# theophile-lt/gpt2-vision-language

Hardware: AMD Instinct MI355X
Metric: training tokens/sec/node, GPT-2-124M seq1024; caption-step images/sec (higher is better)
Workload: dtype bf16; 1 GPU; gpt2-124m-lm-pretrain; micro_batch=16, seq_len=1024, grad_accum=32, global_batch=512, model=gpt2-124m, parallelism=dp1

## Files before the change

gpt2-vision-language_amd/csrc/gemm_pp3.h:

```cpp
#pragma once
#include "common.h"
#include "capi_util.h"
#include "gemm_common.h"
#include "gemm_ring.h"
#include "../../include/gvl.h"

namespace {

using namespace gvl_ring;

template <int PER, int MAXN, int X>
GVL_DEV void wait_vm_steps_x(int n) {
  if (MAXN >= 4 && n >= 4) { asm volatile("s_waitcnt vmcnt(%0)" ::"n"(4 * PER + X) : "memory"); return; }
  if (MAXN >= 3 && n == 3) { asm volatile("s_waitcnt vmcnt(%0)" ::"n"(3 * PER + X) : "memory"); return; }
  if (MAXN >= 2 && n == 2) { asm volatile("s_waitcnt vmcnt(%0)" ::"n"(2 * PER + X) : "memory"); return; }
  if (MAXN >= 1 && n == 1) { asm volatile("s_waitcnt vmcnt(%0)" ::"n"(1 * PER + X) : "memory"); return; }
  asm volatile("s_waitcnt vmcnt(%0)" ::"n"(X) : "memory");
}

constexpr uint32_t CNT_OOB = 0x7FFFFFF0u;
constexpr int CNT_NT = 18;
template <int EPI>
struct CntEpi {
  using KD = EpiKind<EPI>;
  static constexpr bool ON = EPI != EPI_GEN && !KD::AUX && !KD::DROP;
};
template <int FM, int FN, int EPI>
constexpr int cnt_stores() {
  return FM * (FN / 2 + FN % 2) * (EpiKind<EPI>::ACT ? 2 : 1);
}
typedef uint32_t cnt_u32x2 __attribute__((ext_vector_type(2)));
GVL_DEV uint32_t cnt_off(bool ok, int64_t byte_off) {
  uint32_t o = ok ? (uint32_t)byte_off : CNT_OOB;
  asm volatile("" : "+v"(o));
  return o;
}
typedef uint32_t cnt_u32x4 __attribute__((ext_vector_type(4)));

template <int FN>
GVL_DEV void cnt_bias(uint32_t a, uint2 (&bv)[FN]);
template <>
GVL_DEV void cnt_bias<3>(uint32_t a, uint2 (&bv)[3]) {
  asm volatile("ds_read_b64 %0, %3\n\tds_read_b64 %1, %3 offset:32\n\tds_read_b64 %2, %3 offset:64\n\t"
               "s_waitcnt lgkmcnt(0)"
               : "=&v"(bv[0]), "=&v"(bv[1]), "=&v"(bv[2])
               : "v"(a));
}
template <>
GVL_DEV void cnt_bias<4>(uint32_t a, uint2 (&bv)[4]) {
  asm volatile("ds_read_b64 %0, %4\n\tds_read_b64 %1, %4 offset:32\n\tds_read_b64 %2, %4 offset:64\n\t"
               "ds_read_b64 %3, %4 offset:96\n\ts_waitcnt lgkmcnt(0)"
               : "=&v"(bv[0]), "=&v"(bv[1]), "=&v"(bv[2]), "=&v"(bv[3])
               : "v"(a));
}

template <int FM, int FN, int EPI, int AUX>
GVL_DEV void gemm_epilogue_cnt(const GemmP& p, const float4_t (&acc)[FM][FN], int64_t mw0,
                               int64_t nw0, int lane, float alpha, uint32_t bias_lds,
                               __amdgpu_buffer_rsrc_t rc, __amdgpu_buffer_rsrc_t rp) {
  using KD = EpiKind<EPI>;
  const int q = lane >> 4;
  uint2 bv[FN];
#pragma unroll
  for (int j = 0; j < FN; ++j) bv[j] = make_uint2(0, 0);
  if constexpr (KD::BIAS) cnt_bias<FN>(bias_lds + (uint32_t)(2 * (nw0 + 4 * q)), bv);
  const uint2 z = make_uint2(0, 0);
#pragma unroll
  for (int i = 0; i < FM; ++i) {
    const int64_t m = mw0 + i * 16 + (lane & 15);
    const bool mok = m < p.M;
#pragma unroll
    for (int j = 0; j + 1 < FN; j += 2) {
      const int64_t n0 = nw0 + j * 16 + 4 * q, n1 = n0 + 16;
      float v0[4], v1[4], h0[4] = {0.f, 0.f, 0.f, 0.f}, h1[4] = {0.f, 0.f, 0.f, 0.f};
      gemm_epi_vals_k<EPI>(p, acc[i][j], m, n0, alpha, 1.f, bv[j], z, v0, h0);
      gemm_epi_vals_k<EPI>(p, acc[i][j + 1], m, n1, alpha, 1.f, bv[j + 1], z, v1, h1);
      const auto sx = __builtin_amdgcn_permlane16_swap(pack2(v0[0], v0[1]), pack2(v1[0], v1[1]), false, false);
      const auto sy = __builtin_amdgcn_permlane16_swap(pack2(v0[2], v0[3]), pack2(v1[2], v1[3]), false, false);
      const int64_t n = nw0 + 16 * (j + (q & 1)) + 8 * (q >> 1);
      const bool ok = mok && n < p.N;
      __builtin_amdgcn_raw_buffer_store_b128(cnt_u32x4{sx[0], sy[0], sx[1], sy[1]}, rc,
                                             cnt_off(ok, (m * p.ldc + n) * 2), 0, AUX);
      if constexpr (KD::ACT) {
        const auto hx = __builtin_amdgcn_permlane16_swap(pack2(h0[0], h0[1]), pack2(h1[0], h1[1]), false, false);
        const auto hy = __builtin_amdgcn_permlane16_swap(pack2(h0[2], h0[3]), pack2(h1[2], h1[3]), false, false);
        __builtin_amdgcn_raw_buffer_store_b128(cnt_u32x4{hx[0], hy[0], hx[1], hy[1]}, rp,
                                               cnt_off(ok, (m * p.ldp + n) * 2), 0, AUX);
      }
    }
    if constexpr (FN % 2 == 1) {
      constexpr int j = FN - 1;
      const int64_t n0 = nw0 + j * 16 + 4 * q;
      float v0[4], h0[4] = {0.f, 0.f, 0.f, 0.f};
      gemm_epi_vals_k<EPI>(p, acc[i][j], m, n0, alpha, 1.f, bv[j], z, v0, h0);
      const bool ok = mok && n0 < p.N;
      __builtin_amdgcn_raw_buffer_store_b64(cnt_u32x2{pack2(v0[0], v0[1]), pack2(v0[2], v0[3])}, rc,
                                            cnt_off(ok, (m * p.ldc + n0) * 2), 0, AUX);
      if constexpr (KD::ACT)
        __builtin_amdgcn_raw_buffer_store_b64(cnt_u32x2{pack2(h0[0], h0[1]), pack2(h0[2], h0[3])}, rp,
                                              cnt_off(ok, (m * p.ldp + n0) * 2), 0, AUX);
    }
  }
}

template <int BN, bool BMN>
struct SlabB {
  using type = Step<256, BMN, 8>;
};
template <bool BMN>
struct SlabB<192, BMN> {
  using type = Step192<BMN>;
};

template <int NS, bool AMN, bool BMN, int EPI, int BN = 256, int BM = 256>
__global__ __launch_bounds__(512, 1) void gemm_pp3_kernel(GemmP p) {
  constexpr int NW = 8, FM = BM / 32, FN = BN / 64;
  static_assert(NS >= 3 && NS <= 6, "ring geometry");
  static_assert(BN == 256 || BN == 192, "tile width");
  static_assert(BM == 256 || BM == 128, "tile height");
  using SA = Step<BM, AMN, NW>;
  using SB = typename SlabB<BN, BMN>::type;
  constexpr int SLOT = SA::BYTES + SB::BYTES;
  constexpr int IPW0 = SA::PER + SB::PER;
  constexpr int IPW1 = SA::PER + (BN == 256 ? SB::PER : 1);
  extern __shared__ __attribute__((aligned(16))) char smem[];
  const int tid = threadIdx.x, lane = tid & 63;
  const int wave = __builtin_amdgcn_readfirstlane(tid >> 6);
  const int g = wave >> 2, wc = wave & 3;

  const int per_batch = p.tiles_m * p.tiles_n * p.splits;
  const int total = per_batch * p.batch;
  const int G = gridDim.x, b = blockIdx.x;
  const int ntl = (total - b + G - 1) / G;
  const int nks = (int)(p.kper / KS);
  const int nsteps = ntl * nks;
  auto tile_coords = [&](int t, int64_t& m0, int64_t& n0, int64_t& k0, int& split, int& bi) {
    const int vid = b + t * G;
    const int q8 = total >> 3, r8 = total & 7, xcd = vid & 7;
    int work = (xcd < r8 ? xcd * (q8 + 1) : r8 * (q8 + 1) + (xcd - r8) * q8) + (vid >> 3);
    bi = work / per_batch;
    work -= bi * per_batch;
    int tm, tn;
    gemm_tile_of(work, p.splits, p.tiles_m, p.tiles_n, p.group, split, tm, tn);
    m0 = (int64_t)tm * BM;
    n0 = (int64_t)tn * BN;
    k0 = (int64_t)split * p.kper;
  };

  const int64_t a_rows = AMN ? p.K : p.M, b_rows = BMN ? p.K : p.N;
  __amdgpu_buffer_rsrc_t ra = uniform_rsrc(p.A, a_rows * p.lda * 2);
  __amdgpu_buffer_rsrc_t rb = uniform_rsrc(p.B, b_rows * p.ldb * 2);
  const int sa_step = SA::step_bytes(p.lda), sb_step = SB::step_bytes(p.ldb);
  int is_t = 0, is_k = 0;
  int offa[SA::PER], offb[SB::PER];
  {
    int64_t m0, n0, k0;
    int sp, bi;
    tile_coords(0, m0, n0, k0, sp, bi);
    if (p.batch > 1) {
      ra = uniform_rsrc(p.Ab[bi], a_rows * p.lda * 2);
      rb = uniform_rsrc(p.Bb[bi], b_rows * p.ldb * 2);
    }
    SA::base_offsets(p.lda, m0, k0, wave, lane, offa);
    SB::base_offsets(p.ldb, n0, k0, wave, lane, offb);
  }

#define GVL_PP3_ISSUE(gstep)                                                        \
  do {                                                                              \
    if ((gstep) < nsteps) {                                                         \
      char* slot_ = smem + ((gstep) % NS) * SLOT;                                   \
      SA::issue_at(ra, offa, is_k * sa_step, slot_, wave);                          \
      SB::issue_at(rb, offb, is_k * sb_step, slot_ + SA::BYTES, wave);              \
      if (++is_k == nks) {                                                          \
        is_k = 0;                                                                   \
        if (++is_t < ntl) {                                                         \
          int64_t m0_, n0_, k0_;                                                    \
          int sp_, bi_;                                                             \
          tile_coords(is_t, m0_, n0_, k0_, sp_, bi_);                               \
          if (p.batch > 1) {                                                        \
            ra = uniform_rsrc(p.Ab[bi_], a_rows * p.lda * 2);                       \
            rb = uniform_rsrc(p.Bb[bi_], b_rows * p.ldb * 2);                       \
          }                                                                         \
          SA::base_offsets(p.lda, m0_, k0_, wave, lane, offa);                      \
          SB::base_offsets(p.ldb, n0_, k0_, wave, lane, offb);                      \
        }                                                                           \
      }                                                                             \
    }                                                                               \
  } while (0)

  float4_t acc[FM][FN];
#pragma unroll
  for (int i = 0; i < FM; ++i)
#pragma unroll
    for (int j = 0; j < FN; ++j) acc[i][j] = float4_t{0.f, 0.f, 0.f, 0.f};

  const int arow = g * (BM / 2), bcol = wc * (BN / 4);
  constexpr bool DB = EPI == EPI_RES && AMN && BMN;
  constexpr int FPW = FM / 4 > 0 ? FM / 4 : 1;
  float4_t bacc[DB ? FPW : 1];
#pragma unroll
  for (int k = 0; k < (DB ? FPW : 1); ++k) bacc[k] = float4_t{0.f, 0.f, 0.f, 0.f};
  short8_t ones;
#pragma unroll
  for (int k = 0; k < 8; ++k) ones[k] = (short)0x3F80;
  bool do_db = false;
  constexpr bool CNT = CntEpi<EPI>::ON;
  constexpr int CNT_S = cnt_stores<FM, FN, EPI>();
  static_assert(!CNT || (NS - 2) * (IPW0 > IPW1 ? IPW0 : IPW1) + CNT_S <= 63, "vmcnt range");
  const bool cnt_on = CNT && p.cnt;
  const uint32_t bias_lds = (uint32_t)(NS * SLOT);
  const __amdgpu_buffer_rsrc_t rc_cnt = uniform_rsrc(p.C, CNT ? p.M * p.ldc * 2 : 0);
  const __amdgpu_buffer_rsrc_t rp_cnt =
      uniform_rsrc(EpiKind<EPI>::ACT ? p.pre_out : p.C, CNT && EpiKind<EPI>::ACT ? p.M * p.ldp * 2 : 0);
  if constexpr (CNT && EpiKind<EPI>::BIAS) {
    if (cnt_on)
      for (int n = tid * 8; n < p.N; n += 512 * 8)
        *reinterpret_cast<uint4*>(smem + NS * SLOT + 2 * n) = *reinterpret_cast<const uint4*>(p.bias + n);
  }
  int cnt_w = 0;
  float alpha = p.alpha;
  if (p.alpha_ptr) alpha *= *p.alpha_ptr;
#pragma unroll
  for (int i = 0; i < NS - 1; ++i) GVL_PP3_ISSUE(i);
  {
    const int r = nsteps - 1, n = r < 0 ? 0 : (r < NS - 2 ? r : NS - 2);
    if (g == 0) wait_vm_steps<IPW0, NS - 2>(n);
    else wait_vm_steps<IPW1, NS - 2>(n);
  }
  barrier_lds();
  if (g == 1) __builtin_amdgcn_s_barrier();

  int cu_t = 0, cu_k = 0;
  int64_t cu_m0, cu_n0, cu_k0;
  int cu_sp, cu_bi;
  tile_coords(0, cu_m0, cu_n0, cu_k0, cu_sp, cu_bi);
  EpiPre<FM, FN, EPI> pre;
  if (!cnt_on) pre.load_bias(p, cu_n0 + bcol, lane);
  if constexpr (DB) do_db = p.batch > 1 && p.splits == 1 && cu_n0 == 0 && p.Db[cu_bi] != nullptr;
#define GVL_PP3_EPILOGUE()                                                                   \
  do {                                                                                       \
    bool epi_ = true;                                                                        \
    if (p.splits == 2 && p.tickets != nullptr) {     \
         \
      const int tile_ = (cu_bi * p.tiles_m + (int)(cu_m0 / BM)) * p.tiles_n + (int)(cu_n0 / BN); \
      const int64_t pofs_ = (int64_t)cu_bi * 2 * p.M * p.N;                                  \
      const __amdgpu_buffer_rsrc_t rw = uniform_rsrc(p.ws + pofs_, p.ws_bytes - pofs_ * 4);   \
      epi_ = gemm_splitk_arrive<FM, FN>(p, acc, cu_sp, tile_, wave, cu_m0 + arow,            \
                                        cu_n0 + bcol, lane, rw);                             \
      if (epi_) gemm_splitk_gather<FM, FN>(p, acc, cu_sp, cu_m0 + arow, cu_n0 + bcol, lane, rw); \
    } else if (p.splits > 1) {                                                               \
      gemm_store_partial<FM, FN>(p, acc, cu_sp, cu_m0 + arow, cu_n0 + bcol, lane);           \
      epi_ = false;                                                                          \
    }                                                                                        \
    if (epi_) {                                                                              \
      void* c_ = p.batch > 1 ? p.Cb[cu_bi] : p.C;                                           \
      if (CNT && cnt_on) {                                                                   \
        if (p.st_nt)                                                                         \
          gemm_epilogue_cnt<FM, FN, EPI, CNT_NT>(p, acc, cu_m0 + arow, cu_n0 + bcol, lane, alpha, \
                                                 bias_lds, rc_cnt, rp_cnt);                  \
        else                                                                                 \
          gemm_epilogue_cnt<FM, FN, EPI, 0>(p, acc, cu_m0 + arow, cu_n0 + bcol, lane, alpha,  \
                                            bias_lds, rc_cnt, rp_cnt);                       \
        cnt_w = NS - 2;                                                                      \
      } else {                                                                               \
        gemm_epilogue16<FM, FN, EPI>(p, acc, cu_m0 + arow, cu_n0 + bcol, lane, alpha, pre, c_, \
                                     p.batch > 1 ? static_cast<const bf16_t*>(c_) : p.residual); \
      }                                                                                      \
    }                                                                                        \
    if constexpr (DB) {                                                                      \
      if (do_db && (lane >> 4) == 0) {                                                       \
        bf16_t* db_ = static_cast<bf16_t*>(p.Db[cu_bi]);                                     \
        _Pragma("unroll") for (int k = 0; k < FPW; ++k) {                                    \
          const int64_t m_ = cu_m0 + arow + 16 * (wc * FPW + k) + lane;                      \
          if (m_ < p.M) db_[m_] = f2bf(bf2f(db_[m_]) + bacc[k][0] * alpha);                  \
        }                                                                                    \
      }                                                                                      \
      _Pragma("unroll") for (int k = 0; k < FPW; ++k) bacc[k] = float4_t{0.f, 0.f, 0.f, 0.f}; \
    }                                                                                        \
  } while (0)

  short8_t af[FM], bf[FN];
  for (int c = 0; c < nsteps; ++c) {
    if (cu_k == 0 && c > 0) {
      GVL_PP3_EPILOGUE();
#pragma unroll
      for (int i = 0; i < FM; ++i)
#pragma unroll
        for (int j = 0; j < FN; ++j) acc[i][j] = float4_t{0.f, 0.f, 0.f, 0.f};
      ++cu_t;
      tile_coords(cu_t, cu_m0, cu_n0, cu_k0, cu_sp, cu_bi);
      if (!cnt_on) pre.load_bias(p, cu_n0 + bcol, lane);
      if constexpr (DB) do_db = p.batch > 1 && p.splits == 1 && cu_n0 == 0 && p.Db[cu_bi] != nullptr;
    }
    const char* sl = smem + (c % NS) * SLOT;
#pragma unroll
    for (int j = 0; j < FN; ++j) bf[j] = SB::frag(sl + SA::BYTES, bcol + 16 * j, lane);
#pragma unroll
    for (int i = 0; i < FM; ++i) af[i] = SA::frag(sl, arow + 16 * i, lane);
    GVL_PP3_ISSUE(c + NS - 1);
    {
      const int r = nsteps - (c + 2);
      const int n_ = r < 0 ? 0 : (r < NS - 2 ? r : NS - 2);
      if (g == 1) {
        if (CNT && cnt_w > 0) {
          wait_vm_steps_x<IPW1, NS - 2, CNT_S>(n_);
          --cnt_w;
        } else {
          wait_vm_steps<IPW1, NS - 2>(n_);
        }
      }
    }
    barrier_lds();
    __builtin_amdgcn_s_setprio(1);
#pragma unroll
    for (int i = 0; i < FM; ++i)
#pragma unroll
      for (int j = 0; j < FN; ++j) acc[i][j] = mfma16(bf[j], af[i], acc[i][j]);
    if constexpr (DB) {
      if (do_db) {
#pragma unroll
        for (int k = 0; k < FPW; ++k) {
          if (wc == 0) bacc[k] = mfma16(ones, af[k], bacc[k]);
          else if (wc == 1) bacc[k] = mfma16(ones, af[(FPW + k) % FM], bacc[k]);
          else if (wc == 2) bacc[k] = mfma16(ones, af[(2 * FPW + k) % FM], bacc[k]);
          else bacc[k] = mfma16(ones, af[(3 * FPW + k) % FM], bacc[k]);
        }
      }
    }
    __builtin_amdgcn_s_setprio(0);
    if (++cu_k == nks) cu_k = 0;
    {
      const int r = nsteps - (c + 2);
      const int n_ = r < 0 ? 0 : (r < NS - 2 ? r : NS - 2);
      if (g == 0) {
        if (CNT && cnt_w > 0) {
          wait_vm_steps_x<IPW0, NS - 2, CNT_S>(n_);
          --cnt_w;
        } else {
          wait_vm_steps<IPW0, NS - 2>(n_);
        }
      }
    }
    barrier_lds();
  }
#undef GVL_PP3_ISSUE
  if (g == 0) __builtin_amdgcn_s_barrier();
  if (nsteps > 0) GVL_PP3_EPILOGUE();
#undef GVL_PP3_EPILOGUE
}

template <int NS, bool AMN, bool BMN, int EPI, int BN, int BM>
int launch_pp3_bn(const GemmP& p0, const gvl::GemmSink& k) {
  if (gvl::gemm_name_only(k, "gemm_pp3_kernel<%d, %s, %s, %d, %d, %d>", NS, gvl::tf(AMN), gvl::tf(BMN), EPI,
                          BN, BM))
    return 0;
  hipStream_t s = k.stream;
  GemmP p = p0;
  constexpr int ring = NS * (BM + BN) * KS * 2;
  const int64_t bias_bytes = EpiKind<EPI>::BIAS ? 2 * (int64_t)p.tiles_n * BN : 0;
  p.cnt = CntEpi<EPI>::ON && p.batch == 1 && ring + bias_bytes <= 160 * 1024 &&
          p.M * p.ldc * 2 <= (int64_t)CNT_OOB &&
          (!EpiKind<EPI>::ACT || (p.pre_out != nullptr && p.M * p.ldp * 2 <= (int64_t)CNT_OOB)) &&
          (!EpiKind<EPI>::BIAS || ((reinterpret_cast<uintptr_t>(p.bias) & 15) == 0 && p.N % 8 == 0));
  p.st_nt = p.cnt &&p.M * p.ldc * 2 > (int64_t)1 << 30;
  const int lds = ring + (p.cnt ? (int)bias_bytes : 0);
  auto kern = gemm_pp3_kernel<NS, AMN, BMN, EPI, BN, BM>;
  static bool attr_set = false;
  if (!attr_set) {
    (void)hipFuncSetAttribute((const void*)kern, hipFuncAttributeMaxDynamicSharedMemorySize, 160 * 1024);
    attr_set = true;
  }
  const int total = p.tiles_m * p.tiles_n * p.splits * p.batch;
  const int grid = total < gvl::num_cus() ? total : gvl::num_cus();
  gvl::launch_timed(kern, dim3(grid), dim3(512), lds, s, p);
  if (p.splits > 1 && !(p.splits == 2 && p.tickets)) gvl::gemm_splitk_reduce_launch(p, s);
  return 0;
}

constexpr int PP3_NS = 4;
template <int NS, bool AMN, bool BMN, int EPI>
int launch_pp3(const GemmP& p, const gvl::GemmSink& s) {
  if (p.bm == 128) return launch_pp3_bn<NS, AMN, BMN, EPI, 192, 128>(p, s);
  return p.bn == 192 ? launch_pp3_bn<NS, AMN, BMN, EPI, 192, 256>(p, s)
                     : launch_pp3_bn<NS, AMN, BMN, EPI, 256, 256>(p, s);
}

template <int NS, bool AMN, bool BMN>
int launch_pp3_epi(const GemmP& p, const gvl::GemmSink& s) {
  if (p.splits > 1 && !(p.splits == 2 && p.tickets)) return launch_pp3<NS, AMN, BMN, EPI_PLAIN>(p, s);
  switch (gvl::gemm_epi_kind(p)) {
    case EPI_PLAIN: return launch_pp3<NS, AMN, BMN, EPI_PLAIN>(p, s);
    case EPI_BIAS: return launch_pp3<NS, AMN, BMN, EPI_BIAS>(p, s);
    case EPI_BIAS_RES: return launch_pp3<NS, AMN, BMN, EPI_BIAS_RES>(p, s);
    case EPI_BIAS_ACT: return launch_pp3<NS, AMN, BMN, EPI_BIAS_ACT>(p, s);
    case EPI_DACT: return launch_pp3<NS, AMN, BMN, EPI_DACT>(p, s);
    case EPI_RES: return launch_pp3<NS, AMN, BMN, EPI_RES>(p, s);
    case EPI_BIAS_ACT_ERF: return launch_pp3<NS, AMN, BMN, EPI_BIAS_ACT_ERF>(p, s);
    case EPI_DACT_ERF: return launch_pp3<NS, AMN, BMN, EPI_DACT_ERF>(p, s);
    case EPI_BIAS_ACT_D: return launch_pp3<NS, AMN, BMN, EPI_BIAS_ACT_D>(p, s);
    case EPI_BIAS_ACT_ERF_D: return launch_pp3<NS, AMN, BMN, EPI_BIAS_ACT_ERF_D>(p, s);
    case EPI_MUL: return launch_pp3<NS, AMN, BMN, EPI_MUL>(p, s);
    case EPI_BIAS_DROP_RES: return launch_pp3<NS, AMN, BMN, EPI_BIAS_DROP_RES>(p, s);
    case EPI_BIAS_QGELU: return launch_pp3<NS, AMN, BMN, EPI_BIAS_QGELU>(p, s);
    default: return -1;
  }
}

}
```

gpt2-vision-language_amd/csrc/gemm_ring.h:

```cpp
#pragma once
#include "common.h"

namespace gvl_ring {

constexpr int KS = 32;
typedef __attribute__((address_space(3))) void lds_void_t;

GVL_DEV int f64b(int row) { return (row >> 1) & 2; }
GVL_DEV int fT(int k) { return ((k & 3) | ((k >> 1) & 4)) << 1; }

GVL_DEV __amdgpu_buffer_rsrc_t uniform_rsrc(const void* base, int64_t bytes) {
  const uint64_t a = reinterpret_cast<uint64_t>(base);
  const uint32_t lo = __builtin_amdgcn_readfirstlane((uint32_t)a);
  const uint32_t hi = __builtin_amdgcn_readfirstlane((uint32_t)(a >> 32));
  const int n = __builtin_amdgcn_readfirstlane((int)(bytes < 0x7fffffff ? bytes : 0x7fffffff));
  return __builtin_amdgcn_make_buffer_rsrc(
      reinterpret_cast<void*>(((uint64_t)hi << 32) | lo), 0, n, 0x00020000);
}

template <int R, bool MN, int NWV>
struct Step {
  static constexpr int BYTES = R * KS * 2;
  static constexpr int NINSTR = BYTES / 1024;

  GVL_DEV static void issue(__amdgpu_buffer_rsrc_t rs, int64_t ld, int64_t r0, int64_t k0,
                            char* lds, int wave, int lane) {
#pragma unroll
    for (int t = 0; t < NINSTR / NWV; ++t) {
      const int j = t * NWV + wave;
      int64_t off_elems;
      if (!MN) {
        const int row = 16 * j + (lane >> 2);
        const int lc = (lane & 3) ^ f64b(row);
        off_elems = (r0 + row) * ld + k0 + lc * 8;
      } else {
        const int half = j >> 3, kr = 4 * (j & 7) + (lane >> 4);
        const int lc = (lane & 15) ^ fT(kr);
        off_elems = (k0 + kr) * ld + r0 + half * 128 + lc * 8;
      }
      __builtin_amdgcn_raw_ptr_buffer_load_lds(rs, (lds_void_t*)(lds + j * 1024), 16,
                                               (int)(off_elems * 2), 0, 0, 0);
    }
  }

  static constexpr int PER = NINSTR / NWV;
  GVL_DEV static void base_offsets(int64_t ld, int64_t r0, int64_t k0, int wave, int lane,
                                   int (&off)[PER]) {
#pragma unroll
    for (int t = 0; t < PER; ++t) {
      const int j = t * NWV + wave;
      int64_t e;
      if (!MN) {
        const int row = 16 * j + (lane >> 2);
        e = (r0 + row) * ld + k0 + ((lane & 3) ^ f64b(row)) * 8;
      } else {
        const int half = j >> 3, kr = 4 * (j & 7) + (lane >> 4);
        e = (k0 + kr) * ld + r0 + half * 128 + ((lane & 15) ^ fT(kr)) * 8;
      }
      off[t] = (int)(e * 2);
    }
  }
  GVL_DEV static int step_bytes(int64_t ld) { return MN ? (int)(KS * ld * 2) : KS * 2; }
  GVL_DEV static void issue_at(__amdgpu_buffer_rsrc_t rs, const int (&off)[PER], int kbytes,
                               char* lds, int wave) {
#pragma unroll
    for (int t = 0; t < PER; ++t) {
      const int j = t * NWV + wave;
      __builtin_amdgcn_raw_ptr_buffer_load_lds(rs, (lds_void_t*)(lds + j * 1024), 16, off[t],
                                               kbytes, 0, 0);
    }
  }

  GVL_DEV static short8_t frag(const char* lds, int c0, int lane) {
    if (!MN) {
      const int row = c0 + (lane & 15), ch = lane >> 4;
      return *reinterpret_cast<const short8_t*>(lds + row * 64 + ((ch ^ f64b(row)) << 4));
    } else {
      const int G = lane >> 4, i = lane & 15, q = i >> 2, p = i & 3;
      const int half = c0 >> 7, cl = c0 & 127;
      const int kr = 8 * G + q;
      const int ch = (cl >> 3) + (p >> 1);
      const char* base = lds + half * (KS * 256);
      const int off1 = kr * 256 + ((ch ^ fT(kr)) << 4) + (p & 1) * 8;
      short8_t r;
      r.lo = lds_read_tr(base + off1);
      r.hi = lds_read_tr(base + off1 + 4 * 256);
      return r;
    }
  }
};

GVL_DEV int f2(int k) { return (((k >> 1) & 1) | ((k >> 2) & 2)) << 1; }

template <bool MN, int NWV = 8>
struct Step192 {
  static constexpr int R = 192;
  static constexpr int BYTES = R * KS * 2;
  static constexpr int NINSTR = BYTES / 1024;
  static constexpr int PER = (NINSTR + NWV - 1) / NWV;
  GVL_DEV static int64_t elem(int64_t ld, int64_t r0, int64_t k0, int j, int lane) {
    if (!MN) {
      const int row = 16 * j + (lane >> 2);
      return (r0 + row) * ld + k0 + ((lane & 3) ^ f64b(row)) * 8;
    }
    if (j < 8) {
      const int kr = 4 * j + (lane >> 4);
      return (k0 + kr) * ld + r0 + ((lane & 15) ^ fT(kr)) * 8;
    }
    const int kr = 8 * (j - 8) + (lane >> 3);
    return (k0 + kr) * ld + r0 + 128 + ((lane & 7) ^ f2(kr)) * 8;
  }
  GVL_DEV static void base_offsets(int64_t ld, int64_t r0, int64_t k0, int wave, int lane,
                                   int (&off)[PER]) {
#pragma unroll
    for (int t = 0; t < PER; ++t) {
      const int j = t * NWV + wave;
      off[t] = j < NINSTR ? (int)(elem(ld, r0, k0, j, lane) * 2) : 0;
    }
  }
  GVL_DEV static int step_bytes(int64_t ld) { return MN ? (int)(KS * ld * 2) : KS * 2; }
  GVL_DEV static void issue_at(__amdgpu_buffer_rsrc_t rs, const int (&off)[PER], int kbytes,
                               char* lds, int wave) {
#pragma unroll
    for (int t = 0; t < PER; ++t) {
      const int j = t * NWV + wave;
      if (j < NINSTR)
        __builtin_amdgcn_raw_ptr_buffer_load_lds(rs, (lds_void_t*)(lds + j * 1024), 16, off[t],
                                                 kbytes, 0, 0);
    }
  }
  GVL_DEV static short8_t frag(const char* lds, int c0, int lane) {
    if (!MN) {
      const int row = c0 + (lane & 15), ch = lane >> 4;
      return *reinterpret_cast<const short8_t*>(lds + row * 64 + ((ch ^ f64b(row)) << 4));
    }
    const int G = lane >> 4, i = lane & 15, q = i >> 2, p = i & 3;
    const int kr = 8 * G + q;
    short8_t r;
    if (c0 < 128) {
      const int ch = (c0 >> 3) + (p >> 1);
      const int off1 = kr * 256 + ((ch ^ fT(kr)) << 4) + (p & 1) * 8;
      r.lo = lds_read_tr(lds + off1);
      r.hi = lds_read_tr(lds + off1 + 4 * 256);
    } else {
      const int ch = ((c0 - 128) >> 3) + (p >> 1);
      const char* base = lds + 8192;
      const int off1 = kr * 128 + ((ch ^ f2(kr)) << 4) + (p & 1) * 8;
      r.lo = lds_read_tr(base + off1);
      r.hi = lds_read_tr(base + off1 + 4 * 128);
    }
    return r;
  }
};

template <int PER, int MAXN>
GVL_DEV void wait_vm_steps(int n) {
  if (MAXN >= 4 && n >= 4) { asm volatile("s_waitcnt vmcnt(%0)" ::"n"(4 * PER) : "memory"); return; }
  if (MAXN >= 3 && n == 3) { asm volatile("s_waitcnt vmcnt(%0)" ::"n"(3 * PER) : "memory"); return; }
  if (MAXN >= 2 && n == 2) { asm volatile("s_waitcnt vmcnt(%0)" ::"n"(2 * PER) : "memory"); return; }
  if (MAXN >= 1 && n == 1) { asm volatile("s_waitcnt vmcnt(%0)" ::"n"(1 * PER) : "memory"); return; }
  asm volatile("s_waitcnt vmcnt(0)" ::: "memory");
}

GVL_DEV void barrier_lds() {
  asm volatile("s_waitcnt lgkmcnt(0)" ::: "memory");
  __builtin_amdgcn_s_barrier();
}

}
```

gpt2-vision-language_amd/csrc/gemm_w4x.hip:

```cpp
#include "common.h"
#include "capi_util.h"
#include "gemm_common.h"
#include "gemm_ring.h"
#include "../../include/gvl.h"

namespace {

using namespace gvl_ring;

template <int BM>
constexpr int x_ns() { return BM == 256 ? 5 : 7; }

#if defined(__HIP_DEVICE_COMPILE__)
#define W4X_MFMA(acc, bfr, afr) \
  asm volatile("v_mfma_f32_16x16x32_bf16 %0, %1, %2, %0" : "+a"(acc) : "v"(bfr), "v"(afr))
#define W4X_PIN(acc) asm volatile("" : "+a"(acc))
#else
#define W4X_MFMA(acc, bfr, afr) (void)0
#define W4X_PIN(acc) (void)0
#endif

template <int FM, int FN>
GVL_DEV void w4x_fence(float4_t (&acc)[FM][FN]) {
  asm volatile("s_nop 7\n\ts_nop 7\n\ts_nop 7" ::: "memory");
#pragma unroll
  for (int i = 0; i < FM; ++i)
#pragma unroll
    for (int j = 0; j < FN; ++j) W4X_PIN(acc[i][j]);
}

GVL_DEV void w4x_piece(__amdgpu_buffer_rsrc_t r, char* lds, int voff, int soff) {
  __builtin_amdgcn_raw_ptr_buffer_load_lds(r, (lds_void_t*)lds, 16, voff, soff, 0, 0);
}

GVL_DEV short8_t w4x_frag_bmn(const char* slab, int c0, int lane) {
  const int G = lane >> 4, i = lane & 15, q = i >> 2, pp = i & 3;
  const int kr = 8 * G + q;
  const int h = c0 >> 7;
  const int ch = ((c0 - 128 * h) >> 3) + (pp >> 1);
  const int pitch = 256 >> h;
  const int sw = fT(kr) + (f2(kr) - fT(kr)) * h;
  const uint32_t o1 = (uint32_t)reinterpret_cast<uintptr_t>(slab) + 8192 * h + kr * pitch +
                      ((ch ^ sw) << 4) + (pp & 1) * 8;
  const uint32_t o2 = o1 + 4 * pitch;
  short4_t lo, hv;
  asm volatile("ds_read_b64_tr_b16 %0, %2\n\tds_read_b64_tr_b16 %1, %3"
               : "=&v"(lo), "=&v"(hv) : "v"(o1), "v"(o2) : "memory");
  short8_t r;
  r.lo = lo;
  r.hi = hv;
  return r;
}
GVL_DEV short8_t w4x_frag_amn(const char* slab, int c0, int lane) {
  const int G = lane >> 4, i = lane & 15, q = i >> 2, pp = i & 3;
  const int kr = 8 * G + q;
  const int ch = ((c0 & 127) >> 3) + (pp >> 1);
  const uint32_t o1 = (uint32_t)reinterpret_cast<uintptr_t>(slab) + (c0 >> 7) * (KS * 256) + kr * 256 +
                      ((ch ^ fT(kr)) << 4) + (pp & 1) * 8;
  const uint32_t o2 = o1 + 4 * 256;
  short4_t lo, hv;
  asm volatile("ds_read_b64_tr_b16 %0, %2\n\tds_read_b64_tr_b16 %1, %3"
               : "=&v"(lo), "=&v"(hv) : "v"(o1), "v"(o2) : "memory");
  short8_t r;
  r.lo = lo;
  r.hi = hv;
  return r;
}

template <int FM, int FN>
GVL_DEV void w4x_wait(short8_t (&a)[FM], short8_t (&b)[FN]);
template <>
GVL_DEV void w4x_wait<8, 8>(short8_t (&a)[8], short8_t (&b)[8]) {
  asm volatile("s_waitcnt lgkmcnt(0)"
               : "+v"(a[0]), "+v"(a[1]), "+v"(a[2]), "+v"(a[3]), "+v"(a[4]), "+v"(a[5]), "+v"(a[6]),
                 "+v"(a[7]), "+v"(b[0]), "+v"(b[1]), "+v"(b[2]), "+v"(b[3]), "+v"(b[4]), "+v"(b[5]),
                 "+v"(b[6]), "+v"(b[7])
               :
               : "memory");
}
template <>
GVL_DEV void w4x_wait<8, 6>(short8_t (&a)[8], short8_t (&b)[6]) {
  asm volatile("s_waitcnt lgkmcnt(0)"
               : "+v"(a[0]), "+v"(a[1]), "+v"(a[2]), "+v"(a[3]), "+v"(a[4]), "+v"(a[5]), "+v"(a[6]),
                 "+v"(a[7]), "+v"(b[0]), "+v"(b[1]), "+v"(b[2]), "+v"(b[3]), "+v"(b[4]), "+v"(b[5])
               :
               : "memory");
}
template <>
GVL_DEV void w4x_wait<4, 6>(short8_t (&a)[4], short8_t (&b)[6]) {
  asm volatile("s_waitcnt lgkmcnt(0)"
               : "+v"(a[0]), "+v"(a[1]), "+v"(a[2]), "+v"(a[3]), "+v"(b[0]), "+v"(b[1]), "+v"(b[2]),
                 "+v"(b[3]), "+v"(b[4]), "+v"(b[5])
               :
               : "memory");
}

template <int BN, bool MN>
struct XSlabB {
  using type = Step192<MN, 4>;
};
template <bool MN>
struct XSlabB<256, MN> {
  using type = Step<256, MN, 4>;
};


template <int BM, int BN, bool AMN, bool BMN, int EPI, bool GR>
GVL_DEV void gemm_w4x_body(const GemmP& p) {
  constexpr int NS = x_ns<BM>(), FM = BM / 32, FN = BN / 32;
  using SA = Step<BM, AMN, 4>;
  using SB = typename XSlabB<BN, BMN>::type;
  constexpr int SLOT = SA::BYTES + SB::BYTES;
  constexpr int PER = SA::PER + SB::PER;
  static_assert(SA::PER * 4 == SA::NINSTR && SB::PER * 4 == SB::NINSTR, "piece split");
  static_assert(NS * SLOT <= 160 * 1024, "LDS");
  static_assert((NS - 2) * PER <= 63, "vmcnt range");
  extern __shared__ __attribute__((aligned(16))) char smem[];
  const int tid = threadIdx.x, lane = tid & 63;
  const int wave = __builtin_amdgcn_readfirstlane(tid >> 6);
  const int arow = (wave >> 1) * (BM / 2), bcol = (wave & 1) * (BN / 2);
  const int per_batch = p.tiles_m * p.tiles_n;
  const int total = GR ? p.gtile[p.batch] : per_batch * p.batch;
  const int G = gridDim.x;
  __amdgpu_buffer_rsrc_t ra = uniform_rsrc(p.A, (AMN ? p.K : p.M) * p.lda * 2);
  __amdgpu_buffer_rsrc_t rb = uniform_rsrc(p.B, (BMN ? p.K : p.N) * p.ldb * 2);
  constexpr bool DB = EPI == EPI_RES && AMN && BMN && BM == 256;
  float4_t bacc[4];
  short8_t ones;
#pragma unroll
  for (int k = 0; k < 8; ++k) ones[k] = (short)0x3F80;
  const uint32_t db_hi = (wave & 1) ? 0xFFFFFFFFu : 0u;
  const float alpha_dev = p.alpha_ptr ? *p.alpha_ptr : 1.f;
  const float alpha_all = GR ? p.alpha : p.alpha * alpha_dev;

  float4_t acc[FM][FN];
  short8_t fa[2][FM], fb[2][FN];
  int offa[SA::PER], offb[SB::PER];

  for (int vid = blockIdx.x; vid < total; vid += G) {
    const int q8 = total >> 3, r8 = total & 7, xcd = vid & 7;
    const int work = (xcd < r8 ? xcd * (q8 + 1) : r8 * (q8 + 1) + (xcd - r8) * q8) + (vid >> 3);
    int bi, local, tiles_m = p.tiles_m, tiles_n = p.tiles_n;
    int64_t M_ = p.M, N_ = p.N, K_ = p.K, lda_ = p.lda, ldb_ = p.ldb, ldc_ = p.ldc;
    if constexpr (GR) {
      bi = 0;
      while (bi + 1 < p.batch && work >= p.gtile[bi + 1]) ++bi;
      local = work - p.gtile[bi];
      M_ = p.Mb[bi], N_ = p.Nb[bi], K_ = p.Kb[bi], lda_ = p.ldab[bi], ldb_ = p.ldbb[bi], ldc_ = p.ldcb[bi];
      tiles_m = (int)((M_ + BM - 1) / BM);
      tiles_n = (int)((N_ + BN - 1) / BN);
    } else {
      bi = work / per_batch;
      local = work - bi * per_batch;
    }
    const int nks = (int)(K_ / KS);
    const int64_t a_rows = AMN ? K_ : M_, b_rows = BMN ? K_ : N_;
    const int sa_step = SA::step_bytes(lda_), sb_step = SB::step_bytes(ldb_);
    int split, tm, tn;
    gemm_tile_of(local, 1, tiles_m, tiles_n, p.group, split, tm, tn);
    const int64_t m0 = (int64_t)tm * BM, n0 = (int64_t)tn * BN;
    const bool multi = GR || p.batch > 1;
    void* const cout = multi ? p.Cb[bi] : p.C;
    const bf16_t* const res = multi ? static_cast<const bf16_t*>(p.Cb[bi]) : p.residual;
    if (multi) {
      ra = uniform_rsrc(p.Ab[bi], a_rows * lda_ * 2);
      rb = uniform_rsrc(p.Bb[bi], b_rows * ldb_ * 2);
    }
    const float alpha = GR && ((p.alpha_mask >> bi) & 1) ? alpha_all * alpha_dev : alpha_all;
    bool do_db = false;
    if constexpr (DB) do_db = multi && n0 == 0 && p.Db[bi] != nullptr;
    SA::base_offsets(lda_, m0, 0, wave, lane, offa);
    SB::base_offsets(ldb_, n0, 0, wave, lane, offb);
    EpiPre<FM, FN, EPI> pre;
    pre.load_bias(p, n0 + bcol, lane);
    const int aux_at = nks >= 2 ? nks - 2 : 0;
    constexpr bool FOLD = EPI == EPI_BIAS_RES && !GR && !AMN;
    uint2 rx[FOLD ? FM : 1][FOLD ? FN : 1];
    if constexpr (FOLD) {
#pragma unroll
      for (int i = 0; i < FM; ++i) {
        const int64_t m = m0 + arow + 16 * i + (lane & 15);
#pragma unroll
        for (int j = 0; j < FN; ++j) {
          const int64_t n = n0 + bcol + 16 * j + 4 * (lane >> 4);
          rx[i][j] = (m < p.M && n < p.N) ? *reinterpret_cast<const uint2*>(res + m * p.ldr + n)
                                          : make_uint2(0, 0);
        }
      }
    }

#define W4X_PIECE_A(t, step) \
  w4x_piece(ra, smem + ((step) % NS) * SLOT + ((t) * 4 + wave) * 1024, offa[t], (step) * sa_step)
#define W4X_PIECE_B(t, step)                                                                  \
  w4x_piece(rb, smem + ((step) % NS) * SLOT + SA::BYTES + ((t) * 4 + wave) * 1024, offb[t],    \
            (step) * sb_step)

#pragma unroll
    for (int s = 0; s < NS - 1; ++s) {
      if (s < nks) {
#pragma unroll
        for (int t = 0; t < SA::PER; ++t) W4X_PIECE_A(t, s);
#pragma unroll
        for (int t = 0; t < SB::PER; ++t) W4X_PIECE_B(t, s);
      }
    }
#pragma unroll
    for (int i = 0; i < FM; ++i)
#pragma unroll
      for (int j = 0; j < FN; ++j) {
        if constexpr (FOLD) {
          const uint2 v = rx[i][j];
          acc[i][j] = float4_t{lo_bf(v.x), hi_bf(v.x), lo_bf(v.y), hi_bf(v.y)};
        } else {
          acc[i][j] = float4_t{0.f, 0.f, 0.f, 0.f};
        }
      }
    if constexpr (DB) {
#pragma unroll
      for (int k = 0; k < 4; ++k) bacc[k] = float4_t{0.f, 0.f, 0.f, 0.f};
    }
// ... 215 lines not shown
```

Baseline: 952,800 tokens/s.

## Extend counted-store epilogue to MUL aux epilogues with prefetched aux loads

```diff
diff --git a/gpt2-vision-language_amd/csrc/gemm_pp3.h b/gpt2-vision-language_amd/csrc/gemm_pp3.h
--- a/gpt2-vision-language_amd/csrc/gemm_pp3.h
+++ b/gpt2-vision-language_amd/csrc/gemm_pp3.h
@@ -23,7 +23,8 @@
 template <int EPI>
 struct CntEpi {
   using KD = EpiKind<EPI>;
-  static constexpr bool ON = EPI != EPI_GEN && !KD::AUX && !KD::DROP;
+  static constexpr bool AUXL = KD::MUL;
+  static constexpr bool ON = EPI != EPI_GEN && (!KD::AUX || AUXL) && !KD::DROP;
 };
 template <int FM, int FN, int EPI>
 constexpr int cnt_stores() {
@@ -100,6 +101,128 @@
         __builtin_amdgcn_raw_buffer_store_b64(cnt_u32x2{pack2(h0[0], h0[1]), pack2(h0[2], h0[3])}, rp,
                                               cnt_off(ok, (m * p.ldp + n0) * 2), 0, AUX);
     }
+  }
+}
+
+template <int FN>
+constexpr int cnt_aux_row() {
+  return FN / 2 + FN % 2;
+}
+template <int FM, int FN>
+constexpr int cnt_aux_pre() {
+  return FM == 8 && FN == 4 ? 0 : FM / 2;
+}
+template <int FN, int R>
+struct CntAux {
+  cnt_u32x4 x[R > 0 ? R : 1][FN / 2 > 0 ? FN / 2 : 1];
+  cnt_u32x2 y[FN % 2 == 1 && R > 0 ? R : 1];
+};
+typedef uint32_t cnt_rsrc_w __attribute__((ext_vector_type(4)));
+template <int FN, int R, bool ASM>
+GVL_DEV void cnt_aux_load(const GemmP& p, CntAux<FN, R>& a, int64_t mw0, int64_t nw0, int lane,
+                          int i0, __amdgpu_buffer_rsrc_t rx, cnt_rsrc_w rw) {
+  const int q = lane >> 4;
+#pragma unroll
+  for (int i = 0; i < R; ++i) {
+    const int64_t m = mw0 + (i0 + i) * 16 + (lane & 15);
+    const bool mok = m < p.M;
+#pragma unroll
+    for (int j = 0; j + 1 < FN; j += 2) {
+      const int64_t n = nw0 + 16 * (j + (q & 1)) + 8 * (q >> 1);
+      const uint32_t o = cnt_off(mok && n < p.N, (m * p.ldp + n) * 2);
+      if constexpr (ASM)
+        asm volatile("buffer_load_dwordx4 %0, %1, %2, 0 offen" : "=v"(a.x[i][j / 2]) : "v"(o), "s"(rw) : "memory");
+      else
+        a.x[i][j / 2] = __builtin_amdgcn_raw_buffer_load_b128(rx, o, 0, 0);
+    }
+    if constexpr (FN % 2 == 1) {
+      const int64_t n0 = nw0 + (FN - 1) * 16 + 4 * q;
+      const uint32_t o = cnt_off(mok && n0 < p.N, (m * p.ldp + n0) * 2);
+      if constexpr (ASM)
+        asm volatile("buffer_load_dwordx2 %0, %1, %2, 0 offen" : "=v"(a.y[i]) : "v"(o), "s"(rw) : "memory");
+      else
+        a.y[i] = __builtin_amdgcn_raw_buffer_load_b64(rx, o, 0, 0);
+    }
+  }
+}
+template <int N, int FN, int R>
+GVL_DEV void cnt_aux_wait(CntAux<FN, R>& a) {
+  asm volatile("s_waitcnt vmcnt(%0)" : : "n"(N) : "memory");
+#pragma unroll
+  for (int i = 0; i < R; ++i) {
+#pragma unroll
+    for (int j = 0; j < FN / 2; ++j) asm volatile("" : "+v"(a.x[i][j]));
+    if constexpr (FN % 2 == 1) asm volatile("" : "+v"(a.y[i]));
+  }
+}
+template <int FM, int FN, int EPI, int AUX, int R>
+GVL_DEV void gemm_epilogue_cnt_aux_rows(const GemmP& p, const float4_t (&acc)[FM][FN], int64_t mw0,
+                                        int64_t nw0, int lane, float alpha, int i0,
+                                        const CntAux<FN, R>& a, __amdgpu_buffer_rsrc_t rc) {
+  const int q = lane >> 4;
+  const uint2 z = make_uint2(0, 0);
+#pragma unroll
+  for (int ii = 0; ii < R; ++ii) {
+    const int i = i0 + ii;
+    const int64_t m = mw0 + i * 16 + (lane & 15);
+    const bool mok = m < p.M;
+#pragma unroll
+    for (int j = 0; j + 1 < FN; j += 2) {
+      const int64_t n0 = nw0 + j * 16 + 4 * q, n1 = n0 + 16;
+      const cnt_u32x4 l = a.x[ii][j / 2];
+      const auto ax = __builtin_amdgcn_permlane16_swap(l[0], l[2], false, false);
+      const auto ay = __builtin_amdgcn_permlane16_swap(l[1], l[3], false, false);
+      float v0[4], v1[4], h0[4] = {0.f, 0.f, 0.f, 0.f}, h1[4] = {0.f, 0.f, 0.f, 0.f};
+      gemm_epi_vals_k<EPI>(p, acc[i][j], m, n0, alpha, 1.f, z, make_uint2(ax[0], ay[0]), v0, h0);
+      gemm_epi_vals_k<EPI>(p, acc[i][j + 1], m, n1, alpha, 1.f, z, make_uint2(ax[1], ay[1]), v1, h1);
+      const auto sx = __builtin_amdgcn_permlane16_swap(pack2(v0[0], v0[1]), pack2(v1[0], v1[1]), false, false);
+      const auto sy = __builtin_amdgcn_permlane16_swap(pack2(v0[2], v0[3]), pack2(v1[2], v1[3]), false, false);
+      const int64_t n = nw0 + 16 * (j + (q & 1)) + 8 * (q >> 1);
+      __builtin_amdgcn_raw_buffer_store_b128(cnt_u32x4{sx[0], sy[0], sx[1], sy[1]}, rc,
+                                             cnt_off(mok && n < p.N, (m * p.ldc + n) * 2), 0, AUX);
+    }
+    if constexpr (FN % 2 == 1) {
+      constexpr int j = FN - 1;
+      const int64_t n0 = nw0 + j * 16 + 4 * q;
+      float v0[4], h0[4] = {0.f, 0.f, 0.f, 0.f};
+      gemm_epi_vals_k<EPI>(p, acc[i][j], m, n0, alpha, 1.f, z, make_uint2(a.y[ii][0], a.y[ii][1]), v0, h0);
+      __builtin_amdgcn_raw_buffer_store_b64(cnt_u32x2{pack2(v0[0], v0[1]), pack2(v0[2], v0[3])}, rc,
+                                            cnt_off(mok && n0 < p.N, (m * p.ldc + n0) * 2), 0, AUX);
+    }
+  }
+}
+template <int FM, int FN, int EPI, int AUX, int P0, int P1>
+GVL_DEV void gemm_epilogue_cnt_aux(const GemmP& p, const float4_t (&acc)[FM][FN], int64_t mw0,
+                                   int64_t nw0, int lane, float alpha,
+                                   CntAux<FN, cnt_aux_pre<FM, FN>()>& a0, int after,
+                                   __amdgpu_buffer_rsrc_t rc, __amdgpu_buffer_rsrc_t rx) {
+  constexpr int PRE = cnt_aux_pre<FM, FN>(), L1 = (FM - PRE) * cnt_aux_row<FN>();
+  static_assert(L1 + (P0 > P1 ? P0 : P1) <= 63, "vmcnt range");
+  asm volatile("" : "+v"(lane));
+  if constexpr (PRE > 0) {
+    CntAux<FN, FM - PRE> a1;
+    cnt_aux_load<FN, FM - PRE, false>(p, a1, mw0, nw0, lane, PRE, rx, cnt_rsrc_w{0, 0, 0, 0});
+    if (after == 0) cnt_aux_wait<L1>(a0);
+    else if (P0 == P1 || after == P0) cnt_aux_wait<L1 + P0>(a0);
+    else cnt_aux_wait<L1 + P1>(a0);
+    gemm_epilogue_cnt_aux_rows<FM, FN, EPI, AUX, PRE>(p, acc, mw0, nw0, lane, alpha, 0, a0, rc);
+    gemm_epilogue_cnt_aux_rows<FM, FN, EPI, AUX, FM - PRE>(p, acc, mw0, nw0, lane, alpha, PRE, a1, rc);
+  } else {
+#pragma unroll
+    for (int h = 0; h < 2; ++h) {
+      CntAux<FN, FM / 2> a1;
+      cnt_aux_load<FN, FM / 2, false>(p, a1, mw0, nw0, lane, h * (FM / 2), rx, cnt_rsrc_w{0, 0, 0, 0});
+      gemm_epilogue_cnt_aux_rows<FM, FN, EPI, AUX, FM / 2>(p, acc, mw0, nw0, lane, alpha, h * (FM / 2), a1, rc);
+    }
+  }
+}
+template <int PER, int MAXN, int U, int EMAX, int E = 0>
+GVL_DEV void wait_vm_steps_e(int n, int e) {
+  if constexpr (E + U > EMAX) {
+    wait_vm_steps_x<PER, MAXN, E>(n);
+  } else {
+    if (e <= E) wait_vm_steps_x<PER, MAXN, E>(n);
+    else wait_vm_steps_e<PER, MAXN, U, EMAX, E + U>(n, e);
   }
 }
 
@@ -218,6 +341,26 @@
         *reinterpret_cast<uint4*>(smem + NS * SLOT + 2 * n) = *reinterpret_cast<const uint4*>(p.bias + n);
   }
   int cnt_w = 0;
+  constexpr bool CNTA = CNT && CntEpi<EPI>::AUXL;
+  constexpr int APRE = cnt_aux_pre<FM, FN>(), AU = APRE * cnt_aux_row<FN>();
+  constexpr int XU = APRE > 0 ? AU : CNT_S, XMAX = 2 * (CNT_S + AU);
+  static_assert(!CNTA || (CNT_S % XU == 0 && (NS - 2) * (IPW0 > IPW1 ? IPW0 : IPW1) + XMAX <= 63),
+                "vmcnt range");
+  constexpr bool TRA = CNTA && AMN, TRB = CNTA && BMN;
+  CntAux<FN, APRE> aux0;
+  const __amdgpu_buffer_rsrc_t rx_cnt = uniform_rsrc(CNTA ? p.pre_in : p.A, CNTA ? p.M * p.ldp * 2 : 0);
+  cnt_rsrc_w rw_cnt = {0, 0, 0, 0};
+  if constexpr (CNTA) {
+    const uint64_t a_ = reinterpret_cast<uint64_t>(p.pre_in);
+    const int64_t n_ = p.M * p.ldp * 2;
+    rw_cnt = cnt_rsrc_w{(uint32_t)__builtin_amdgcn_readfirstlane((int)(uint32_t)a_),
+                        (uint32_t)__builtin_amdgcn_readfirstlane((int)(uint32_t)(a_ >> 32)),
+                        (uint32_t)__builtin_amdgcn_readfirstlane((int)(n_ < 0x7fffffff ? n_ : 0x7fffffff)),
+                        0x00020000u};
+  }
+  const int aux_at = nks >= 2 ? nks - 2 : 0;
+  int aux_after = 0;
+  int x_cur = 0, x_prev = 0;
   float alpha = p.alpha;
   if (p.alpha_ptr) alpha *= *p.alpha_ptr;
 #pragma unroll
@@ -248,14 +391,22 @@
       epi_ = gemm_splitk_arrive<FM, FN>(p, acc, cu_sp, tile_, wave, cu_m0 + arow,            \
                                         cu_n0 + bcol, lane, rw);                             \
       if (epi_) gemm_splitk_gather<FM, FN>(p, acc, cu_sp, cu_m0 + arow, cu_n0 + bcol, lane, rw); \
-    } else if (p.splits > 1) {                                                               \
+    } else if (!CNTA && p.splits > 1) {      \
       gemm_store_partial<FM, FN>(p, acc, cu_sp, cu_m0 + arow, cu_n0 + bcol, lane);           \
       epi_ = false;                                                                          \
     }                                                                                        \
     if (epi_) {                                                                              \
       void* c_ = p.batch > 1 ? p.Cb[cu_bi] : p.C;                                           \
-      if (CNT && cnt_on) {                                                                   \
+      if (CNTA && cnt_on) {                                                                  \
         if (p.st_nt)                                                                         \
+          gemm_epilogue_cnt_aux<FM, FN, EPI, CNT_NT, IPW0, IPW1>(                            \
+              p, acc, cu_m0 + arow, cu_n0 + bcol, lane, alpha, aux0, aux_after, rc_cnt, rx_cnt); \
+        else                                                                                 \
+          gemm_epilogue_cnt_aux<FM, FN, EPI, 0, IPW0, IPW1>(                                 \
+              p, acc, cu_m0 + arow, cu_n0 + bcol, lane, alpha, aux0, aux_after, rc_cnt, rx_cnt); \
+        x_cur += CNT_S;                                     \
+      } else if (CNT && cnt_on) {                                                            \
+        if (p.st_nt)                                                                      \
           gemm_epilogue_cnt<FM, FN, EPI, CNT_NT>(p, acc, cu_m0 + arow, cu_n0 + bcol, lane, alpha, \
                                                  bias_lds, rc_cnt, rp_cnt);                  \
         else                                                                                 \
@@ -281,6 +432,10 @@
 
   short8_t af[FM], bf[FN];
   for (int c = 0; c < nsteps; ++c) {
+    if constexpr (CNTA) {
+      x_prev = x_cur;
+      x_cur = 0;
+    }
     if (cu_k == 0 && c > 0) {
       GVL_PP3_EPILOGUE();
 #pragma unroll
@@ -294,21 +449,41 @@
     }
     const char* sl = smem + (c % NS) * SLOT;
 #pragma unroll
-    for (int j = 0; j < FN; ++j) bf[j] = SB::frag(sl + SA::BYTES, bcol + 16 * j, lane);
-#pragma unroll
-    for (int i = 0; i < FM; ++i) af[i] = SA::frag(sl, arow + 16 * i, lane);
+    for (int j = 0; j < FN; ++j)
+      bf[j] = TRB ? (BN == 192 ? frag_tr192_asm(sl + SA::BYTES, bcol + 16 * j, lane)
+                               : frag_tr_asm(sl + SA::BYTES, bcol + 16 * j, lane))
+                  : SB::frag(sl + SA::BYTES, bcol + 16 * j, lane);
+#pragma unroll
+    for (int i = 0; i < FM; ++i) af[i] = TRA ? frag_tr_asm(sl, arow + 16 * i, lane) : SA::frag(sl, arow + 16 * i, lane);
     GVL_PP3_ISSUE(c + NS - 1);
+    if constexpr (CNTA) {
+      if (APRE > 0 && cnt_on && cu_k == aux_at) {
+        int lane_ = lane;
+        asm volatile("" : "+v"(lane_));
+        cnt_aux_load<FN, APRE, true>(p, aux0, cu_m0 + arow, cu_n0 + bcol, lane_, 0, rx_cnt, rw_cnt);
+        x_cur += AU;
+        aux_after = nks >= 2 && c + 1 + NS - 1 < nsteps ? (g == 0 ? IPW0 : IPW1) : 0;
+      }
+    }
     {
       const int r = nsteps - (c + 2);
       const int n_ = r < 0 ? 0 : (r < NS - 2 ? r : NS - 2);
       if (g == 1) {
-        if (CNT && cnt_w > 0) {
+        if (CNTA && cnt_on) {
+          wait_vm_steps_e<IPW1, NS - 2, XU, XMAX>(n_, x_prev + x_cur);
+        } else if (CNT && cnt_w > 0) {
           wait_vm_steps_x<IPW1, NS - 2, CNT_S>(n_);
           --cnt_w;
         } else {
           wait_vm_steps<IPW1, NS - 2>(n_);
         }
       }
+    }
+    if constexpr (TRA || TRB) {
+#pragma unroll
+      for (int j = 0; j < (TRB ? FN : 0); ++j) asm volatile("s_waitcnt lgkmcnt(0)" : "+v"(bf[j]) : : "memory");
+#pragma unroll
+      for (int i = 0; i < (TRA ? FM : 0); ++i) asm volatile("s_waitcnt lgkmcnt(0)" : "+v"(af[i]) : : "memory");
     }
     barrier_lds();
     __builtin_amdgcn_s_setprio(1);
@@ -333,7 +508,9 @@
       const int r = nsteps - (c + 2);
       const int n_ = r < 0 ? 0 : (r < NS - 2 ? r : NS - 2);
       if (g == 0) {
-        if (CNT && cnt_w > 0) {
+        if (CNTA && cnt_on) {
+          wait_vm_steps_e<IPW0, NS - 2, XU, XMAX>(n_, x_prev + x_cur);
+        } else if (CNT && cnt_w > 0) {
           wait_vm_steps_x<IPW0, NS - 2, CNT_S>(n_);
           --cnt_w;
         } else {
@@ -360,6 +537,8 @@
   const int64_t bias_bytes = EpiKind<EPI>::BIAS ? 2 * (int64_t)p.tiles_n * BN : 0;
   p.cnt = CntEpi<EPI>::ON && p.batch == 1 && ring + bias_bytes <= 160 * 1024 &&
           p.M * p.ldc * 2 <= (int64_t)CNT_OOB &&
+          (!CntEpi<EPI>::AUXL || (p.splits == 1 && (reinterpret_cast<uintptr_t>(p.pre_in) & 15) == 0 &&
+                                  p.ldp % 8 == 0 && p.M * p.ldp * 2 <= (int64_t)CNT_OOB)) &&
           (!EpiKind<EPI>::ACT || (p.pre_out != nullptr && p.M * p.ldp * 2 <= (int64_t)CNT_OOB)) &&
           (!EpiKind<EPI>::BIAS || ((reinterpret_cast<uintptr_t>(p.bias) & 15) == 0 && p.N % 8 == 0));
   p.st_nt = p.cnt &&p.M * p.ldc * 2 > (int64_t)1 << 30;
diff --git a/gpt2-vision-language_amd/csrc/gemm_ring.h b/gpt2-vision-language_amd/csrc/gemm_ring.h
--- a/gpt2-vision-language_amd/csrc/gemm_ring.h
+++ b/gpt2-vision-language_amd/csrc/gemm_ring.h
@@ -153,6 +153,40 @@
   }
 };
 
+GVL_DEV short8_t frag_tr192_asm(const char* slab, int c0, int lane) {
+  const int G = lane >> 4, i = lane & 15, q = i >> 2, pp = i & 3;
+  const int kr = 8 * G + q;
+  const int h = c0 >> 7;
+  const int ch = ((c0 - 128 * h) >> 3) + (pp >> 1);
+  const int pitch = 256 >> h;
+  const int sw = fT(kr) + (f2(kr) - fT(kr)) * h;
+  const uint32_t o1 = (uint32_t)reinterpret_cast<uintptr_t>(slab) + 8192 * h + kr * pitch +
+                      ((ch ^ sw) << 4) + (pp & 1) * 8;
+  const uint32_t o2 = o1 + 4 * pitch;
+  short4_t lo, hv;
+  asm volatile("ds_read_b64_tr_b16 %0, %2\n\tds_read_b64_tr_b16 %1, %3"
+               : "=&v"(lo), "=&v"(hv) : "v"(o1), "v"(o2) : "memory");
+  short8_t r;
+  r.lo = lo;
+  r.hi = hv;
+  return r;
+}
+GVL_DEV short8_t frag_tr_asm(const char* slab, int c0, int lane) {
+  const int G = lane >> 4, i = lane & 15, q = i >> 2, pp = i & 3;
+  const int kr = 8 * G + q;
+  const int ch = ((c0 & 127) >> 3) + (pp >> 1);
+  const uint32_t o1 = (uint32_t)reinterpret_cast<uintptr_t>(slab) + (c0 >> 7) * (KS * 256) + kr * 256 +
+                      ((ch ^ fT(kr)) << 4) + (pp & 1) * 8;
+  const uint32_t o2 = o1 + 4 * 256;
+  short4_t lo, hv;
+  asm volatile("ds_read_b64_tr_b16 %0, %2\n\tds_read_b64_tr_b16 %1, %3"
+               : "=&v"(lo), "=&v"(hv) : "v"(o1), "v"(o2) : "memory");
+  short8_t r;
+  r.lo = lo;
+  r.hi = hv;
+  return r;
+}
+
 template <int PER, int MAXN>
 GVL_DEV void wait_vm_steps(int n) {
   if (MAXN >= 4 && n >= 4) { asm volatile("s_waitcnt vmcnt(%0)" ::"n"(4 * PER) : "memory"); return; }
diff --git a/gpt2-vision-language_amd/csrc/gemm_w4x.hip b/gpt2-vision-language_amd/csrc/gemm_w4x.hip
--- a/gpt2-vision-language_amd/csrc/gemm_w4x.hip
+++ b/gpt2-vision-language_amd/csrc/gemm_w4x.hip
@@ -33,39 +33,8 @@
   __builtin_amdgcn_raw_ptr_buffer_load_lds(r, (lds_void_t*)lds, 16, voff, soff, 0, 0);
 }
 
-GVL_DEV short8_t w4x_frag_bmn(const char* slab, int c0, int lane) {
-  const int G = lane >> 4, i = lane & 15, q = i >> 2, pp = i & 3;
-  const int kr = 8 * G + q;
-  const int h = c0 >> 7;
-  const int ch = ((c0 - 128 * h) >> 3) + (pp >> 1);
-  const int pitch = 256 >> h;
-  const int sw = fT(kr) + (f2(kr) - fT(kr)) * h;
-  const uint32_t o1 = (uint32_t)reinterpret_cast<uintptr_t>(slab) + 8192 * h + kr * pitch +
-                      ((ch ^ sw) << 4) + (pp & 1) * 8;
-  const uint32_t o2 = o1 + 4 * pitch;
-  short4_t lo, hv;
-  asm volatile("ds_read_b64_tr_b16 %0, %2\n\tds_read_b64_tr_b16 %1, %3"
-               : "=&v"(lo), "=&v"(hv) : "v"(o1), "v"(o2) : "memory");
-  short8_t r;
-  r.lo = lo;
-  r.hi = hv;
-  return r;
-}
-GVL_DEV short8_t w4x_frag_amn(const char* slab, int c0, int lane) {
-  const int G = lane >> 4, i = lane & 15, q = i >> 2, pp = i & 3;
-  const int kr = 8 * G + q;
-  const int ch = ((c0 & 127) >> 3) + (pp >> 1);
-  const uint32_t o1 = (uint32_t)reinterpret_cast<uintptr_t>(slab) + (c0 >> 7) * (KS * 256) + kr * 256 +
-                      ((ch ^ fT(kr)) << 4) + (pp & 1) * 8;
-  const uint32_t o2 = o1 + 4 * 256;
-  short4_t lo, hv;
-  asm volatile("ds_read_b64_tr_b16 %0, %2\n\tds_read_b64_tr_b16 %1, %3"
-               : "=&v"(lo), "=&v"(hv) : "v"(o1), "v"(o2) : "memory");
-  short8_t r;
-  r.lo = lo;
-  r.hi = hv;
-  return r;
-}
+GVL_DEV short8_t w4x_frag_bmn(const char* slab, int c0, int lane) { return frag_tr192_asm(slab, c0, lane); }
+GVL_DEV short8_t w4x_frag_amn(const char* slab, int c0, int lane) { return frag_tr_asm(slab, c0, lane); }
 
 template <int FM, int FN>
 GVL_DEV void w4x_wait(short8_t (&a)[FM], short8_t (&b)[FN]);
```

Measured after the change: 930,100 tokens/s. -2.4%, worse.
